# rishikksh20/FastSpeech2

Hardware: NVIDIA H100
Metric: mel-frames/sec (batched inference) (higher is better)
Workload: dtype 3xf16

## Files before the change

### fastspeech2_b200/_lib.py

```python
from __future__ import annotations

import ctypes as C
import os
from typing import Optional

import torch

_HERE = os.path.dirname(os.path.abspath(__file__))
LIB_PATH = os.path.join(_HERE, "libfs2b200.so")

FS2_DUR_I64, FS2_DUR_F32, FS2_DUR_I32 = 0, 1, 2
FS2_PER_UTTERANCE = 1
MATH_FP32, MATH_TF32, MATH_3XTF32, MATH_F16 = 0, 1, 2, 3
MATH_MODES = {"fp32": MATH_FP32, "tf32": MATH_TF32, "3xtf32": MATH_3XTF32, "3xf16": MATH_3XTF32, "f16": MATH_F16}


class Fs2Error(RuntimeError):
    pass


class Config(C.Structure):
    _fields_ = [(n, C.c_int32) for n in (
        "idim", "odim", "adim", "aheads", "elayers", "eunits", "ddim", "dlayers", "dunits", "ffn_kernel",
        "pred_layers", "pred_chans", "pred_kernel", "postnet_layers", "postnet_chans", "postnet_filts",
# ... 18 lines not shown
SIGNATURES = {
    "fs2_create": [C.POINTER(_P), C.POINTER(Config), _I],
    "fs2_set_math_mode": [_P, _I],
    "fs2_profile_enable": [_P, _I],
    "fs2_profile_classes": [],
    "fs2_profile_read": [_P, C.POINTER(C.c_double), C.POINTER(_L), C.POINTER(C.c_double), C.POINTER(C.c_double)],
    "fs2_load_weights": [_P, C.POINTER(WeightDesc), _I, _P],
    "fs2_workspace_bytes": [_P, _I, _I, _I, C.POINTER(_SZ)],
    "fs2_encode": [_P, _P, _P, _I, _I, _P, _P, _P, _P, _SZ, _P],
    "fs2_encode_ex": [_P, _P, _P, _I, _I, _P, _P, _P, _P, _SZ, _I, _P],
    "fs2_length_plan": [_P, _I, _P, _F, _I, _I, _I, _P, _P, _P, _P],
    "fs2_length_gather": [_P, _P, _P, _I, _I, _I, _P, _I, _P],
    "fs2_length_plan_ex": [_P, _I, _P, _F, _P, _I, _I, _I, _P, _P, _P, _P, _P],
    "fs2_length_gather_ex": [_P, _P, _P, _I, _I, _I, _P, _I, _P, _P, _P],
    "fs2_decode": [_P, _P, _P, _P, _P, _I, _I, _P, _P, _P, _P, _P, _P, _P, _SZ, _P],
    "fs2_decode_ex": [_P, _P, _P, _P, _P, _I, _I, _P, _P, _P, _P, _P, _P, _P, _SZ, _I, _P],
    "fs2_decode_ctl": [_P, _P, _P, _P, _P, _I, _I, _P, _P, _P, _P, _P, _P, _P, _P, _P, _SZ, _I, _P],
    "fs2_masked_losses": [_P, _P, _P, _I, _P, _P, _I, _P, _P, _P, _P, _P, _P, _I, _I, _I, _I, _P, _P, _P],
    "fs2_bucketize": [_P, _P, _I, _L, _P, _P],
    "fs2_one_hot": [_P, _L, _I, _P, _P],
    "fs2_op_tap_gemm": [_I, _P, _I, _I, _I, _P, _P, _I, _I, _I, _P, _P, _P],
    "fs2_op_tap_gemm_ex": [_I, _P, _I, _I, _I, _P, _P, _I, _I, _I, _P, _P, _P, _P, _I, _I, _P, _I, _P],
    "fs2_op_tap_gemm_dil": [_I, _P, _I, _I, _I, _P, _P, _I, _I, _I, _P, _P, _P, _P, _I, _I, _P, _I, _I, _P],
    "fs2_op_attention": [_I, _P, _P, _I, _I, _I, _I, _P, _P],
    "fs2_op_attention_planes": [_I, _P, _P, _I, _P, _I, _I, _I, _I, _P, _P, _P],
    "fs2_op_gemm_layernorm": [_I, _P, _L, _I, _I, _P, _P, _P, _P, _P, _F, _P, _P, _P],
    "fs2_op_layernorm": [_P, _P, _P, _P, _F, _L, _I, _P, _P],
    "fs2_dropout_mask": [_P, _L, _F, C.c_uint64, C.c_uint64, _P],
    "fs2_dropout_apply": [_P, _P, _F, _P, _L, _P],
    "fs2_act_backward": [_P, _P, _I, _P, _L, _P],
    "fs2_relu": [_P, _P, _L, _P],
    "fs2_add": [_P, _P, _P, _L, _P],
    "fs2_colsum": [_P, _L, _I, _P, _P],
    "fs2_conv_forward": [_P, _I, _I, _I, _P, _P, _I, _I, _I, _P, _P, _P, _P],
    "fs2_conv_dgrad": [_P, _I, _I, _I, _P, _I, _I, _P, _P, _P],
    "fs2_conv_wgrad": [_P, _P, _I, _I, _I, _I, _I, _P, _P, _P],
    "fs2_conv_forward_ex": [_P, _I, _I, _I, _P, _P, _I, _I, _I, _P, _P, _P, _I, _P],
    "fs2_conv_dgrad_ex": [_P, _I, _I, _I, _P, _I, _I, _P, _P, _I, _P],
    "fs2_conv_wgrad_tc_ws_bytes": [_I, _I, _I, _I, _I, C.POINTER(_SZ)],
    "fs2_conv_wgrad_tc": [_P, _P, _I, _I, _I, _I, _I, _P, _P, _P, _SZ, _P],
    "fs2_layernorm_backward": [_P, _P, _P, _F, _L, _I, _P, _P, _P, _P],
    "fs2_batchnorm_train": [_P, _L, _I, _P, _P, _F, _F, _I, _P, _P, _P, _P, _P, _P],
    "fs2_batchnorm_backward": [_P, _P, _P, _P, _F, _L, _I, _P, _P, _P, _P, _P],
    "fs2_bgemm": [_P, _L, _L, _L, _L, _P, _L, _L, _L, _L, _P, _L, _L, _L, _L, _I, _I, _I, _I, _I, _F, _P],
    "fs2_attn_softmax": [_P, _P, _P, _F, _I, _I, _I, _P, _P, _P],
    "fs2_attn_softmax_backward": [_P, _P, _P, _F, _I, _I, _I, _P, _P],
# ... 104 lines not shown
```

### fastspeech2_b200/csrc/api.cu

```cuda
#include <stdarg.h>
#include <stdlib.h>
#include <string.h>

#include <atomic>
#include <string>
#include <unordered_map>
#include <vector>

#include "common.cuh"

namespace fs2 {

static thread_local char g_err[512] = "";
std::atomic<unsigned long long> g_kernel_launches{0};
void set_error(const char* fmt, ...) {
  va_list ap;
  va_start(ap, fmt);
  vsnprintf(g_err, sizeof(g_err), fmt, ap);
  va_end(ap);
}

struct Dense {
  const float* w = nullptr;
  const __half* w_hi = nullptr;
// ... 680 lines not shown
    int rc = split_rows(x, K, rows, K, xp, st);
    if (!rc) rc = weight_scale(w, nw, sc, sc + 1, st);
    if (!rc) rc = split_f16(w, w_hi, w_lo, nw, sc, st);
    return rc;
  }
  ~TempPlanes() { if (base) cudaFreeAsync(base, st); }
};
}

int fs2_op_tap_gemm(int math_mode, const float* x, int B, int L, int K, const float* w, const float* bias, int N, int taps,
                    int act, const float* resid, float* out, void* stream) {
  return fs2_op_tap_gemm_ex(math_mode, x, B, L, K, w, bias, N, taps, act, resid, nullptr, out, nullptr, 0, 0, nullptr, 0,
                            stream);
}
int fs2_op_tap_gemm_ex(int math_mode, const float* x, int B, int L, int K, const float* w, const float* bias, int N,
                       int taps, int act, const float* resid, const int64_t* lens, float* out, void* out_planes,
                       int vt_col0, int vt_heads, void* vt, int vt_lpad, void* stream) {
  return fs2_op_tap_gemm_dil(math_mode, x, B, L, K, w, bias, N, taps, act, resid, lens, out, out_planes, vt_col0, vt_heads, vt,
                             vt_lpad, 1, stream);
}
int fs2_op_tap_gemm_dil(int math_mode, const float* x, int B, int L, int K, const float* w, const float* bias, int N,
                        int taps, int act, const float* resid, const int64_t* lens, float* out, void* out_planes,
                        int vt_col0, int vt_heads, void* vt, int vt_lpad, int dil, void* stream) {
  const char* who = "fs2_op_tap_gemm";
  FS2_REQUIRE(math_mode == FS2_MATH_FP32 || math_mode == FS2_MATH_TF32 || math_mode == FS2_MATH_F16 || math_mode == FS2_MATH_3XTF32,
              "%s: unknown math mode %d", who, math_mode);
  const bool planes = math_mode == FS2_MATH_F16 || math_mode == FS2_MATH_3XTF32;
  FS2_REQUIRE(x && w && (out || (planes && (out_planes || vt))), "%s: null argument", who);
  FS2_REQUIRE(B >= 0 && L >= 0 && K > 0 && N > 0 && taps > 0, "%s: bad shape B=%d L=%d K=%d N=%d taps=%d", who, B, L, K, N, taps);
  FS2_REQUIRE(dil == 1 || (dil > 1 && (long)dil * ((taps - 1) / 2) + L < (1L << 30)),
              "%s: need dil >= 1 and dil * (taps - 1) / 2 + L < 2^30 (got dil=%d taps=%d L=%d)", who, dil, taps, L);
  FS2_REQUIRE(!out_planes || planes, "%s: out_planes needs FS2_MATH_F16 or FS2_MATH_3XTF32", who);
  FS2_REQUIRE(!vt || math_mode != FS2_MATH_FP32, "%s: the fp32 family has no transposed V output", who);
  FS2_REQUIRE(!vt || (vt_heads > 0 && vt_col0 >= 0 && vt_col0 < N && (N - vt_col0) % vt_heads == 0 && vt_lpad >= L),
              "%s: transposed V needs 0 <= vt_col0 < N, heads dividing N - vt_col0 and vt_lpad >= L", who);
  Dense d; d.w = w; d.bias = bias; d.N = N; d.K = K; d.taps = taps;
  cudaStream_t st = (cudaStream_t)stream;
  TapGemm g;
  TempPlanes t;
  if (planes) {
    int rc = t.make(x, (long)B * L, K, w, (long)N * K * taps, st);
    if (rc) return rc;
    d.w_hi = t.w_hi; d.w_lo = t.w_lo; d.w_inv = t.sc + 1;
    g = make_gemm_p(d, t.xp, B, L, math_mode == MATH_3XTF32, act, resid, N, out, N);
    planes_out(g, reinterpret_cast<__half*>(out_planes), N, math_mode == MATH_3XTF32);
  } else {
    g = make_gemm(d, x, K, B, L, act, resid, N, out, N);
  }
  if (vt) {
    g.vt_col0 = vt_col0; g.vt_heads = vt_heads; g.vt_dk = (N - vt_col0) / vt_heads; g.vt_lpad = vt_lpad;
    if (planes) g.vtp = reinterpret_cast<__half*>(vt); else g.vt_out = reinterpret_cast<float*>(vt);
  }
  g.dil = dil;
  return dense(masked(g, lens), math_mode, st, P_DEC_W1);
}
int fs2_op_gemm_layernorm(int math_mode, const float* x, int64_t rows, int K, int N, const float* w, const float* bias, const float* resid,
                          const float* gamma, const float* beta, float eps, float* out, float* out_planes, void* stream) {
  FS2_REQUIRE(x && w && gamma && beta && out, "fs2_op_gemm_layernorm: null argument");
  FS2_REQUIRE(rows < (1LL << 31), "fs2_op_gemm_layernorm: too many rows");
  FS2_REQUIRE(math_mode == FS2_MATH_TF32 || math_mode == FS2_MATH_F16 || math_mode == FS2_MATH_3XTF32,
              "fs2_op_gemm_layernorm: tensor-core modes only (FS2_MATH_TF32, FS2_MATH_F16, FS2_MATH_3XTF32)");
  FS2_REQUIRE(N == 384 || (N == 256 && math_mode != FS2_MATH_TF32), "fs2_op_gemm_layernorm: N must be 384 (or 256 in the plane families)");
  cudaStream_t st = (cudaStream_t)stream;
  Dense d; d.w = w; d.bias = bias; d.N = N; d.K = K; d.taps = 1;
  FS2_REQUIRE(!out_planes || math_mode != FS2_MATH_TF32, "fs2_op_gemm_layernorm: the tf32 variant has no plane output in this entry");
  float* y = nullptr;
  __half* op = nullptr;
  FS2_CUDA_CHECK(cudaMallocAsync(&y, (size_t)rows * N * sizeof(float) + 64, st));
  int rc = FS2_OK;
  if (math_mode == FS2_MATH_TF32) {
    rc = dense(make_gemm(d, x, K, 1, (int)rows, ACT_NONE, resid, N, y, N), FS2_MATH_TF32, st, P_DEC_OUT);
  } else {
    TempPlanes t;
    rc = t.make(x, (long)rows, K, w, (long)N * K, st);
    if (!rc) {
      d.w_hi = t.w_hi; d.w_lo = t.w_lo; d.w_inv = t.sc + 1;
// ... 67 lines not shown
```

### fastspeech2_b200/csrc/common.cuh

```cuda
#pragma once
#include <cuda_fp16.h>
#include <cuda_runtime.h>
#include <stdint.h>
#include <stdio.h>
#include <stdlib.h>

#include <atomic>

#include "../../include/fs2_b200.h"

namespace fs2 {

void set_error(const char* fmt, ...);
extern std::atomic<unsigned long long> g_kernel_launches;

#define FS2_CUDA_CHECK(expr)                                                                   \
  do {                                                                                         \
    cudaError_t _e = (expr);                                                                   \
    if (_e != cudaSuccess) {                                                                   \
      fs2::set_error("%s failed at %s:%d: %s", #expr, __FILE__, __LINE__, cudaGetErrorString(_e)); \
      return FS2_ERR_CUDA;                                                                     \
    }                                                                                          \
  } while (0)

// ... 16 lines not shown

constexpr float kPlaneScale = 16.0f;
constexpr float kPlaneInv = 1.0f / 16.0f;

struct TapGemm {
  const float* x; int ldx;
  int B, L, K;
  const float* w;
  const float* bias;
  int N, taps;
  int act;
  const float* resid; int ldr;
  float* out; int ldo;
  float* vt_out = nullptr; int vt_col0 = 0, vt_dk = 0, vt_heads = 0, vt_lpad = 0;
  __half* vtp = nullptr;
  const __half* xp = nullptr;
  const __half* w_hi = nullptr; const __half* w_lo = nullptr;
  const float* w_inv = nullptr;
  float a_inv = 1.0f;
  __half* outp = nullptr; int ldo_p = 0; bool outp_lo = false;
  bool precise = false;
  const int64_t* lens = nullptr;
  int dil = 1;
};
int tap_gemm_fp32(const TapGemm& g, cudaStream_t st);
int tap_gemm_tf32(const TapGemm& g, cudaStream_t st);
int tap_gemm_planes(const TapGemm& g, cudaStream_t st);
int split_f16(const float* src, __half* hi, __half* lo, long n, const float* scale , cudaStream_t st);
int split_rows(const float* x, int ldx, long rows, int K, __half* planes, cudaStream_t st);
int planes_to_rows(const __half* planes, long n, float* out, cudaStream_t st);
int weight_scale(const float* w, long n, float* scale, float* inv, cudaStream_t st);
constexpr int MATH_3XTF32 = FS2_MATH_3XTF32;

struct RowNorm {
  const float* x; int ldx;
  const float* resid; int ldr;
  const float* gamma; const float* beta; float eps;
  int64_t rows; int C;
  float* out; int ldo;
  int relu_after;
  const float* pe; const float* alpha; int L;
  const float* head_w; const float* head_b; float* head_out; int64_t* dur_out;
  const float* head_scale;
  const int64_t* lens;
  __half* split_out;
  int split_lo;
// ... 32 lines not shown
int pack_conv_weight(const float* src, int N, int K, int taps, const float* scale , float* dst,
                     cudaStream_t st);
int pack_transpose(const float* src, int rows, int cols, float* dst, cudaStream_t st);
int fold_batchnorm(const float* gamma, const float* beta, const float* mean, const float* var, float eps, int N,
                   float* scale, float* shift, cudaStream_t st);

__device__ __forceinline__ void pdl_trigger() { asm volatile("griddepcontrol.launch_dependents;" ::: "memory"); }
__device__ __forceinline__ void pdl_wait() { asm volatile("griddepcontrol.wait;" ::: "memory"); }
inline bool pdl_enabled() {
  static int v = -1;
  if (v < 0) { const char* e = getenv("FS2_PDL"); v = e ? atoi(e) : 0; }
  return v != 0;
}
template <typename... KArgs, typename... Args>
inline cudaError_t launch_pdl(void (*kernel)(KArgs...), dim3 grid, dim3 block, size_t smem, cudaStream_t st, Args... args) {
  cudaLaunchConfig_t cfg = {};
  cfg.gridDim = grid; cfg.blockDim = block; cfg.dynamicSmemBytes = smem; cfg.stream = st;
  cudaLaunchAttribute attr[1];
  attr[0].id = cudaLaunchAttributeProgrammaticStreamSerialization;
  attr[0].val.programmaticStreamSerializationAllowed = 1;
  cfg.attrs = attr; cfg.numAttrs = pdl_enabled() ? 1 : 0;
  return cudaLaunchKernelEx(&cfg, kernel, static_cast<KArgs>(args)...);
}

inline int sm_count_current() {
  static int cached[64];
  int dev = 0;
  cudaGetDevice(&dev);
  if (dev < 0 || dev >= 64) dev = 0;
  if (!cached[dev]) {
    int n = 0;
    if (cudaDeviceGetAttribute(&n, cudaDevAttrMultiProcessorCount, dev) != cudaSuccess || n <= 0) n = 132;
    cached[dev] = n;
  }
  return cached[dev];
}

__device__ __forceinline__ uint32_t pack_f16x2_sat(float a, float b) {
  uint32_t r;
  asm("cvt.rn.satfinite.f16x2.f32 %0, %1, %2;" : "=r"(r) : "f"(b), "f"(a));
  return r;
}
__device__ __forceinline__ void split_pair(float a, float b, uint32_t& hi, uint32_t& lo) {
  a *= kPlaneScale; b *= kPlaneScale;
  hi = pack_f16x2_sat(a, b);
  const float2 g = __half22float2(*reinterpret_cast<const __half2*>(&hi));
// ... 34 lines not shown
```

### fastspeech2_b200/csrc/gemm_tc.cu

```cuda
#include <stdlib.h>

#include "tc_common.cuh"

namespace fs2 {
namespace {
using namespace tc;

constexpr int BM = 128;
constexpr int BK = 32;
constexpr int A_BYTES = BM * BK * 4;
constexpr int THREADS = 384;
constexpr int PRODUCER_REGS = 40, CONSUMER_REGS = 232;
constexpr int RING_BUDGET = 227 * 1024 - 1024  - 256 ;

struct TcParams {
  int L, tiles_per_utt;
  int m_tiles, n_tiles;
  int B, full, gn, upt, full_tiles;
  int K, taps, pad, dil;
  const float* bias; const float* resid; int ldr; int act;
  float* out; int ldo;
  float a_inv; const float* w_inv;
  __half* outp; __half* outp_lo; int ldo_p;
  float* vt_out; __half* vtp; __half* vtp_lo; int vt_col0, vt_dk, vt_heads, vt_lpad, vt_L;
  const int64_t* lens;
};

template <int BN, bool PRECISE, bool HALF = false>
struct Cfg {
  static constexpr int B_BYTES = BN * BK * 4;
  static constexpr int STAGE_BYTES = (PRECISE ? 2 : 1) * (A_BYTES + B_BYTES);
  static_assert(!PRECISE || HALF, "the error-compensated family is 3xF16");
  static constexpr int STAGES = (RING_BUDGET / STAGE_BYTES) > 8 ? 8 : (RING_BUDGET / STAGE_BYTES);
  static constexpr size_t SMEM = (size_t)STAGES * STAGE_BYTES + 1024 + 256;
  static constexpr int BKE = HALF ? 2 * BK : BK;
  static constexpr int A_LO = A_BYTES;
  static constexpr int B_HI = PRECISE ? 2 * A_BYTES : A_BYTES;
  static constexpr int B_LO = B_HI + B_BYTES;
  static constexpr uint32_t TX_BYTES = (PRECISE ? 2 : 1) * (A_BYTES + B_BYTES);
  static_assert(BN % 16 == 0 && BN >= 16 && BN <= 128, "tile width: sums of wgmma N = 128 / 64 / 16");
  static_assert(B_BYTES % 1024 == 0, "B stage must keep 1024-byte alignment");
  static_assert(STAGES >= 2, "resources");
};

template <int BN, bool HALF, int C0 = 0>
__device__ __forceinline__ void mma_tile(float* d, uint64_t a, uint64_t b, uint32_t acc) {
  if constexpr (BN - C0 >= 128) {
    if constexpr (HALF) wgmma_f16_n128(d + C0 / 2, a, b + (C0 * 128 >> 4), acc); else wgmma_tf32_n128(d + C0 / 2, a, b + (C0 * 128 >> 4), acc);
// ... 4 lines not shown
  } else if constexpr (BN - C0 >= 16) {
    if constexpr (HALF) wgmma_f16_n16(d + C0 / 2, a, b + (C0 * 128 >> 4), acc); else wgmma_tf32_n16(d + C0 / 2, a, b + (C0 * 128 >> 4), acc);
    mma_tile<BN, HALF, C0 + 16>(d, a, b, acc);
  }
}

template <int BN, bool PRECISE, bool HALF>
__global__ void __launch_bounds__(THREADS, 1)
tap_gemm_tc_kernel(const __grid_constant__ CUtensorMap tmap_a, const __grid_constant__ CUtensorMap tmap_b,
                   const __grid_constant__ CUtensorMap tmap_b_lo, const __grid_constant__ CUtensorMap tmap_a16, TcParams p) {
  using C = Cfg<BN, PRECISE, HALF>;
  extern __shared__ uint8_t smem_raw[];
  uint8_t* tiles = smem_raw + ((1024u - (smem_u32(smem_raw) & 1023u)) & 1023u);
  uint64_t* full_bar = reinterpret_cast<uint64_t*>(tiles + (size_t)C::STAGES * C::STAGE_BYTES);
  uint64_t* empty_bar = full_bar + C::STAGES;

  const int warp = uniform_warp_idx(), lane = threadIdx.x & 31;
  const int kchunks = (p.K + C::BKE - 1) / C::BKE;
  const int steps = p.taps * kchunks;
  const int total_tiles = p.m_tiles * p.n_tiles;

  uint64_t* order_bar = empty_bar + C::STAGES;

  if (threadIdx.x == 0) {
    for (int s = 0; s < C::STAGES; ++s) { mbar_init(&full_bar[s], 1); mbar_init(&empty_bar[s], 4); }
    mbar_init(&order_bar[0], 4); mbar_init(&order_bar[1], 4);
    asm volatile("fence.mbarrier_init.release.cluster;" ::: "memory");
  }
  __syncthreads();
  pdl_wait();

  auto tile_coords = [&](int tile, int& n0, int& b, int& t0, int& packed) -> bool {
    const int mt = tile / p.n_tiles;
    n0 = (tile - mt * p.n_tiles) * BN;
    packed = -1;
    if (p.tiles_per_utt == 0) { b = 0; t0 = mt * BM; }
    else if (mt < p.full_tiles) { b = mt / p.full; t0 = (mt - b * p.full) * BM; }
    else { packed = mt - p.full_tiles; b = packed * p.upt; t0 = p.full * BM; }
    return packed < 0 && p.lens != nullptr && t0 >= p.lens[b];
  };

  if (warp < 4) {
    setmaxnreg_dec<PRODUCER_REGS>();
    if (warp != 0) { pdl_trigger(); return; }
    const uint32_t tiles_addr = smem_u32(tiles), full_addr = smem_u32(full_bar);
    int n = 0;
    for (int tile = blockIdx.x; tile < total_tiles; tile += gridDim.x) {
      int n0, b, t0, packed;
      if (tile_coords(tile, n0, b, t0, packed)) continue;
      int j = 0, kc = 0;
      for (int s = 0; s < steps; ++s, ++n) {
        const int slot = n % C::STAGES, round = n / C::STAGES;
        const int k0 = kc * C::BKE, row = t0 + (j - p.pad) * p.dil;
        const uint32_t st = tiles_addr + (uint32_t)slot * C::STAGE_BYTES, fb = full_addr + (uint32_t)slot * 8u;
        pin_before(st, fb, k0, row);
        mbar_wait(&empty_bar[slot], (round & 1) ^ 1);
        mbar_expect_tx_elect(fb, C::TX_BYTES);
        if (packed < 0) {
          tma_load_3d_elect(st, &tmap_a, fb, k0, row, b);
          if (PRECISE) tma_load_3d_elect(st + C::A_LO, &tmap_a, fb, k0, row, b + p.B);
        } else {
          for (int g = 0; g < 8; ++g) {
            const int u = g / p.gn, gi = g - u * p.gn;
            const bool real = u < p.upt && b + u < p.B;
            const int oob = PRECISE ? 2 * p.B : p.B;
            tma_load_3d_elect(st + g * (16 * 128), &tmap_a16, fb, k0, row + gi * 16, real ? b + u : oob);
            if (PRECISE) tma_load_3d_elect(st + C::A_LO + g * (16 * 128), &tmap_a16, fb, k0, row + gi * 16, real ? b + u + p.B : oob);
          }
        }
        tma_load_3d_elect(st + C::B_HI, &tmap_b, fb, k0, n0, j);
        if (PRECISE) tma_load_3d_elect(st + C::B_LO, &tmap_b_lo, fb, k0, n0, j);
        if (++kc == kchunks) { kc = 0; ++j; }
      }
    }
  } else {
    setmaxnreg_inc<CONSUMER_REGS>();
    const int cg = (warp >> 2) - 1, wq = warp & 3;
    const int r_lo = 16 * wq + (lane >> 2);
    const int act = p.act, ldr = p.ldr, ldo = p.ldo;
    const float* __restrict__ resid = p.resid; float* __restrict__ out = p.out;
    const bool has_res = resid != nullptr;
    const float oscale = p.a_inv * (p.w_inv ? __ldg(p.w_inv) : 1.0f);
    float d[BN];
    int n = 0;
    int k = 0;
    for (int tile = blockIdx.x; tile < total_tiles; tile += gridDim.x, ++k) {
      int n0, b, t0, packed;
      const int tile_steps = tile_coords(tile, n0, b, t0, packed) ? 0 : steps;
      if ((k & 1) != cg) { n += tile_steps; continue; }
      long m[4]; bool row_ok[4], row_zero[4];
#pragma unroll
      for (int i = 0; i < 4; ++i) {
        const int row = 64 * (i >> 1) + r_lo + 8 * (i & 1);
        int bb = b, t = t0 + row;
        bool ok = t < p.L;
        if (packed >= 0) {
          const int g = row >> 4, u = g / p.gn, gi = g - u * p.gn;
          bb += u;
          t = t0 + gi * 16 + (row & 15);
          ok = u < p.upt && bb < p.B && t < p.L;
        }
        m[i] = (long)bb * p.L + t; row_ok[i] = ok;
        row_zero[i] = ok && p.lens != nullptr && t >= p.lens[bb];
        if (has_res && ok) prefetch_l2(resid + m[i] * ldr + n0);
      }
      if (k > 0) mbar_wait(&order_bar[cg], ((k - 1) >> 1) & 1);
// ... 3 lines not shown
        const uint32_t base = smem_u32(tiles + (size_t)slot * C::STAGE_BYTES);
        const uint64_t a_hi = make_sw128_kmajor_desc(base), b_hi = make_sw128_kmajor_desc(base + C::B_HI);
        const uint64_t a_lo = make_sw128_kmajor_desc(base + C::A_LO), b_lo = make_sw128_kmajor_desc(base + C::B_LO);
        constexpr uint64_t HALF_A = (A_BYTES / 2) >> 4;
        mbar_wait(&full_bar[slot], round & 1);
        wgmma_fence();
#pragma unroll
        for (int kk = 0; kk < 4; ++kk) {
#pragma unroll
          for (int hf = 0; hf < 2; ++hf) {
            float* dh = d + hf * (BN / 2);
            if (PRECISE) {
              mma_tile<BN, true>(dh, a_lo + hf * HALF_A + 2 * kk, b_hi + 2 * kk, (s | kk) != 0);
              mma_tile<BN, true>(dh, a_hi + hf * HALF_A + 2 * kk, b_lo + 2 * kk, 1);
              mma_tile<BN, true>(dh, a_hi + hf * HALF_A + 2 * kk, b_hi + 2 * kk, 1);
            } else {
              mma_tile<BN, HALF>(dh, a_hi + hf * HALF_A + 2 * kk, b_hi + 2 * kk, (s | kk) != 0);
            }
          }
        }
        wgmma_commit();
        wgmma_wait<1>();
        pin_regs<BN>(d);
        if (prev >= 0) { __syncwarp(); if (lane == 0) mbar_arrive(&empty_bar[prev]); }
        prev = slot;
      }
      __syncwarp();
      if (lane == 0) mbar_arrive(&order_bar[cg ^ 1]);
      wgmma_wait<0>();
      pin_regs<BN>(d);
      if (prev >= 0) { __syncwarp(); if (lane == 0) mbar_arrive(&empty_bar[prev]); }
      if (tile_steps == 0) {
#pragma unroll
        for (int i = 0; i < BN; ++i) d[i] = 0.f;
      }

      const bool to_vt = (p.vt_out != nullptr || p.vtp != nullptr) && n0 >= p.vt_col0;
#pragma unroll
      for (int i = 0; i < 4; ++i) {
        if (!row_ok[i] || (to_vt && row_zero[i])) continue;
        const long mm = m[i];
        float* dr = d + (i >> 1) * (BN / 2) + 2 * (i & 1);
#pragma unroll
        for (int jj = 0; jj < BN / 8; ++jj) {
          const int col = n0 + 8 * jj + 2 * (lane & 3);
          float v0 = dr[4 * jj], v1 = dr[4 * jj + 1];
          const float b0 = p.bias ? __ldg(p.bias + col) : 0.f, b1 = p.bias ? __ldg(p.bias + col + 1) : 0.f;
          v0 = fmaf(v0, oscale, b0); v1 = fmaf(v1, oscale, b1);
          if (!to_vt) {
            if (act == ACT_RELU) { v0 = fmaxf(v0, 0.f); v1 = fmaxf(v1, 0.f); }
            else if (act == ACT_TANH) { v0 = tanhf(v0); v1 = tanhf(v1); }
            if (has_res) {
              const float2 r = __ldg(reinterpret_cast<const float2*>(resid + mm * ldr + col));
              v0 += r.x; v1 += r.y;
// ... 23 lines not shown
          continue;
        }
#pragma unroll
        for (int jj = 0; jj < BN / 8; ++jj) {
          const int col = n0 + 8 * jj + 2 * (lane & 3);
          const float v0 = dr[4 * jj], v1 = dr[4 * jj + 1];
          if (HALF && p.outp != nullptr) {
            const long off = mm * p.ldo_p + col;
            if (p.outp_lo != nullptr) {
              uint32_t hi, lo;
              split_pair(v0, v1, hi, lo);
              *reinterpret_cast<uint32_t*>(p.outp + off) = hi;
              *reinterpret_cast<uint32_t*>(p.outp_lo + off) = lo;
            } else {
              *reinterpret_cast<uint32_t*>(p.outp + off) = hi_pair(v0, v1);
            }
          }
          if (out != nullptr) *reinterpret_cast<float2*>(out + mm * ldo + col) = make_float2(v0, v1);
        }
      }
    }
  }
  pdl_trigger();
}

__global__ void split_rows_f16_kernel(const float* __restrict__ x, int ldx, long rows, int K, __half* __restrict__ S) {
  pdl_trigger(); pdl_wait();
  const int kq = K >> 2;
  const long quads = rows * kq;
  __half* __restrict__ lo_plane = S + rows * K;
  for (long i = (long)blockIdx.x * blockDim.x + threadIdx.x; i < quads; i += (long)gridDim.x * blockDim.x) {
    const long r = i / kq;
    const int c = (int)(i - r * kq) * 4;
    const float4 v = *reinterpret_cast<const float4*>(x + r * ldx + c);
    uint2 hv, lv;
    split_pair(v.x, v.y, hv.x, lv.x);
    split_pair(v.z, v.w, hv.y, lv.y);
    *reinterpret_cast<uint2*>(S + r * K + c) = hv;
    *reinterpret_cast<uint2*>(lo_plane + r * K + c) = lv;
  }
}

template <int BN, bool PRECISE, bool HALF = false>
int launch(const TapGemm& g, cudaStream_t st) {
  using C = Cfg<BN, PRECISE, HALF>;
  static unsigned long long configured = 0;
  int rc;
  if ((rc = ensure_smem_attr(tap_gemm_tc_kernel<BN, PRECISE, HALF>, C::SMEM, &configured))) return rc;
  TcParams p;
  p.K = g.K; p.taps = g.taps; p.pad = (g.taps - 1) / 2; p.dil = g.dil > 1 ? g.dil : 1;
  p.bias = g.bias; p.resid = g.resid; p.ldr = g.ldr; p.act = g.act; p.out = g.out; p.ldo = g.ldo;
  const long rows = (long)g.B * g.L;
  p.a_inv = HALF ? g.a_inv : 1.0f; p.w_inv = HALF ? g.w_inv : nullptr;
  p.outp = HALF ? g.outp : nullptr; p.ldo_p = g.ldo_p;
  p.outp_lo = (HALF && g.outp && g.outp_lo) ? g.outp + rows * g.ldo_p : nullptr;
  p.vt_out = HALF ? nullptr : g.vt_out; p.vtp = HALF ? g.vtp : nullptr;
  p.vtp_lo = (HALF && g.vtp && g.outp_lo) ? g.vtp + (long)g.B * g.vt_heads * g.vt_dk * g.vt_lpad : nullptr;
  p.vt_col0 = g.vt_col0; p.vt_dk = g.vt_dk; p.vt_heads = g.vt_heads; p.vt_lpad = g.vt_lpad; p.vt_L = g.L;
  p.lens = g.lens;
  CUtensorMap ma, mb, mb_lo, ma16;
  const int esz = HALF ? 2 : 4;
  constexpr int planes = HALF && PRECISE ? 2 : 1;
  const void* xa = HALF ? (const void*)g.xp : (const void*)g.x;
  const uint64_t row_bytes = HALF ? (uint64_t)g.K * 2 : (uint64_t)g.ldx * 4;
  if (g.taps == 1 && g.lens == nullptr) {
    const uint64_t M = (uint64_t)g.B * g.L;
    p.L = (int)M; p.tiles_per_utt = 0;
    p.m_tiles = (int)((M + BM - 1) / BM);
    p.B = 1; p.full = 0; p.gn = 1; p.upt = 1; p.full_tiles = 0;
    if ((rc = make_map(&ma, xa, g.K, M, planes, row_bytes, row_bytes * M, BM, HALF))) return rc;
    ma16 = ma;
  } else {
    p.L = g.L; p.tiles_per_utt = (g.L + BM - 1) / BM;
    p.B = g.B; p.full = g.L / BM;
    int tail = g.L % BM;
    p.gn = tail ? (tail + 15) / 16 : 1;
    p.upt = tail ? 8 / p.gn : 1;
    if (tail && p.upt == 1) { p.full += 1; tail = 0; p.gn = 1; }
    p.full_tiles = p.full * g.B;
    p.m_tiles = p.full_tiles + (tail ? (g.B + p.upt - 1) / p.upt : 0);
    if ((rc = make_map(&ma, xa, g.K, g.L, (uint64_t)g.B * planes, row_bytes, row_bytes * g.L, BM, HALF))) return rc;
    if ((rc = make_map(&ma16, xa, g.K, g.L, (uint64_t)g.B * planes, row_bytes, row_bytes * g.L, 16, HALF))) return rc;
  }
  p.n_tiles = g.N / BN;
  const void* w_hi = HALF ? (const void*)g.w_hi : (const void*)g.w;
  if ((rc = make_map(&mb, w_hi, g.K, g.N, g.taps, (uint64_t)g.K * esz, (uint64_t)g.K * esz * g.N, BN, HALF))) return rc;
  if ((rc = make_map(&mb_lo, PRECISE ? (const void*)g.w_lo : w_hi, g.K, g.N, g.taps, (uint64_t)g.K * esz, (uint64_t)g.K * esz * g.N, BN, HALF))) return rc;
  const int total = p.m_tiles * p.n_tiles;
  const int grid = total < sm_count_current() ? total : sm_count_current();
  FS2_CUDA_CHECK(launch_pdl(tap_gemm_tc_kernel<BN, PRECISE, HALF>, dim3(grid), dim3(THREADS), C::SMEM, st, ma, mb, mb_lo, ma16, p));
  FS2_LAUNCH_CHECK();
  return FS2_OK;
}

int tile_width(int N) { return N % 128 == 0 ? 128 : N % 80 == 0 ? 80 : N % 64 == 0 ? 64 : N % 32 == 0 ? 32 : 16; }

template <bool PRECISE, bool HALF>
int launch_any(const TapGemm& g, cudaStream_t st) {
  switch (tile_width(g.N)) {
    case 128: return launch<128, PRECISE, HALF>(g, st);
    case 80: return launch<80, PRECISE, HALF>(g, st);
    case 64: return launch<64, PRECISE, HALF>(g, st);
    case 32: return launch<32, PRECISE, HALF>(g, st);
    default: return launch<16, PRECISE, HALF>(g, st);
  }
}

int check_output(const TapGemm& g, const char* who) {
  FS2_REQUIRE((g.taps & 1) == 1, "%s: taps must be odd", who);
  FS2_REQUIRE(g.N % 16 == 0, "%s: N (%d) must be a multiple of 16", who, g.N);
  FS2_REQUIRE(!g.resid || g.ldr % 4 == 0, "%s: row strides must be 16-byte multiples", who);
  FS2_REQUIRE(!g.out || (g.ldo % 8 == 0 && (reinterpret_cast<uintptr_t>(g.out) & 31) == 0), "%s: output rows must be 32-byte aligned", who);
  return FS2_OK;
// ... 112 lines not shown
```

### fastspeech2_b200/csrc/tc_common.cuh

```cuda
#pragma once
#include <cuda.h>

#include "common.cuh"

namespace fs2 {
namespace tc {

__device__ __forceinline__ uint32_t smem_u32(const void* p) { return (uint32_t)__cvta_generic_to_shared(p); }

__device__ __forceinline__ void mbar_init(uint64_t* bar, uint32_t count) {
  asm volatile("mbarrier.init.shared::cta.b64 [%0], %1;" ::"r"(smem_u32(bar)), "r"(count) : "memory");
}
__device__ __forceinline__ void mbar_arrive(uint64_t* bar) {
  asm volatile("mbarrier.arrive.shared::cta.b64 _, [%0];" ::"r"(smem_u32(bar)) : "memory");
}
__device__ __forceinline__ void mbar_wait(uint64_t* bar, uint32_t parity) {
  uint32_t ok;
  asm volatile(
      "{\n\t.reg .pred p, q;\n\t.reg .u32 cnt;\n\t"
      "mov.u32 cnt, 0;\n"
      "FS2_WAIT_LOOP:\n\t"
      "mbarrier.try_wait.parity.shared::cta.b64 p, [%1], %2;\n\t"
      "@p bra FS2_WAIT_DONE;\n\t"
      "add.u32 cnt, cnt, 1;\n\t"
      "setp.lt.u32 q, cnt, 4194304;\n\t"
      "@q bra FS2_WAIT_LOOP;\n"
      "FS2_WAIT_DONE:\n\t"
      "selp.u32 %0, 1, 0, p;\n\t}"
      : "=r"(ok) : "r"(smem_u32(bar)), "r"(parity) : "memory");
  if (!ok) __trap();
}
__device__ __forceinline__ int uniform_warp_idx() { return __shfl_sync(0xffffffffu, (int)(threadIdx.x >> 5), 0); }
__device__ __forceinline__ void mbar_expect_tx_elect(uint32_t bar_addr, uint32_t bytes) {
  asm volatile(
      "{\n\t.reg .pred e;\n\t"
      "elect.sync _|e, 0xffffffff;\n\t"
      "@e mbarrier.arrive.expect_tx.shared::cta.b64 _, [%0], %1;\n\t}"
      ::"r"(bar_addr), "r"(bytes) : "memory");
}
__device__ __forceinline__ void tma_load_3d_elect(uint32_t dst_addr, const CUtensorMap* map, uint32_t bar_addr, int c0, int c1, int c2) {
  asm volatile(
      "{\n\t.reg .pred e;\n\t"
      "elect.sync _|e, 0xffffffff;\n\t"
      "@e cp.async.bulk.tensor.3d.shared::cluster.global.mbarrier::complete_tx::bytes [%0], [%1, {%3, %4, %5}], [%2];\n\t}"
      ::"r"(dst_addr), "l"(reinterpret_cast<uint64_t>(map)), "r"(bar_addr), "r"(c0), "r"(c1), "r"(c2)
      : "memory");
}
__device__ __forceinline__ void pin_before(uint32_t a, uint32_t b, int c, int d) { asm volatile("" ::"r"(a), "r"(b), "r"(c), "r"(d)); }
__device__ __forceinline__ void prefetch_l2(const void* p) { asm volatile("prefetch.global.L2 [%0];" ::"l"(p)); }

__device__ __forceinline__ uint64_t make_sw128_kmajor_desc(uint32_t smem_addr) {
  return (uint64_t)((smem_addr & 0x3FFFFu) >> 4) | (1ull << 16) | ((uint64_t)(1024 >> 4) << 32) | (1ull << 62);
}
__device__ __forceinline__ void wgmma_fence() { asm volatile("wgmma.fence.sync.aligned;" ::: "memory"); }
__device__ __forceinline__ void wgmma_commit() { asm volatile("wgmma.commit_group.sync.aligned;" ::: "memory"); }
template <int N>
__device__ __forceinline__ void wgmma_wait() { asm volatile("wgmma.wait_group.sync.aligned %0;" ::"n"(N) : "memory"); }
template <int N>
__device__ __forceinline__ void pin_regs(float* v) {
#pragma unroll
  for (int i = 0; i < N; ++i) asm volatile("" : "+f"(v[i])::"memory");
}
__device__ __forceinline__ void wgmma_f16_n128(float* d, uint64_t a, uint64_t b, uint32_t acc) {
  asm volatile(
      "{\n\t.reg .pred p;\n\tsetp.ne.b32 p, %66, 0;\n\t"
      "wgmma.mma_async.sync.aligned.m64n128k16.f32.f16.f16 {%0, %1, %2, %3, %4, %5, %6, %7, %8, %9, %10, %11, %12, %13, %14, %15, %16, %17, %18, %19, %20, %21, %22, %23, %24, %25, %26, %27, %28, %29, %30, %31, %32, %33, %34, %35, %36, %37, %38, %39, %40, %41, %42, %43, %44, %45, %46, %47, %48, %49, %50, %51, %52, %53, %54, %55, %56, %57, %58, %59, %60, %61, %62, %63}, %64, %65, p, 1, 1, 0, 0;\n\t}"
      : "+f"(d[0]), "+f"(d[1]), "+f"(d[2]), "+f"(d[3]), "+f"(d[4]), "+f"(d[5]), "+f"(d[6]), "+f"(d[7]), "+f"(d[8]), "+f"(d[9]), "+f"(d[10]), "+f"(d[11]), "+f"(d[12]), "+f"(d[13]), "+f"(d[14]), "+f"(d[15]), "+f"(d[16]), "+f"(d[17]), "+f"(d[18]), "+f"(d[19]), "+f"(d[20]), "+f"(d[21]), "+f"(d[22]), "+f"(d[23]), "+f"(d[24]), "+f"(d[25]), "+f"(d[26]), "+f"(d[27]), "+f"(d[28]), "+f"(d[29]), "+f"(d[30]), "+f"(d[31]), "+f"(d[32]), "+f"(d[33]), "+f"(d[34]), "+f"(d[35]), "+f"(d[36]), "+f"(d[37]), "+f"(d[38]), "+f"(d[39]), "+f"(d[40]), "+f"(d[41]), "+f"(d[42]), "+f"(d[43]), "+f"(d[44]), "+f"(d[45]), "+f"(d[46]), "+f"(d[47]), "+f"(d[48]), "+f"(d[49]), "+f"(d[50]), "+f"(d[51]), "+f"(d[52]), "+f"(d[53]), "+f"(d[54]), "+f"(d[55]), "+f"(d[56]), "+f"(d[57]), "+f"(d[58]), "+f"(d[59]), "+f"(d[60]), "+f"(d[61]), "+f"(d[62]), "+f"(d[63])
      : "l"(a), "l"(b), "r"(acc));
}
// ... 103 lines not shown
```

### include/fs2_b200.h

```cpp
#ifndef FS2_H100_H_
#define FS2_H100_H_

#include <stddef.h>
#include <stdint.h>

#ifdef __cplusplus
extern "C" {
#endif

#define FS2_OK 0
#define FS2_ERR_INVALID (-1)
#define FS2_ERR_CUDA (-2)
#define FS2_ERR_MISSING_WEIGHT (-3)
#define FS2_ERR_WORKSPACE (-4)
#define FS2_ERR_NOT_LOADED (-5)

#define FS2_DUR_I64 0
#define FS2_DUR_F32 1
#define FS2_DUR_I32 2

#define FS2_MATH_FP32 0
#define FS2_MATH_TF32 1
#define FS2_MATH_3XTF32 2
#define FS2_MATH_F16 3
// ... 62 lines not shown
int fs2_decode_ex(fs2_handle* h, const float* hm, const int64_t* olens, const float* es, const float* ps, int B, int L,
                  float* before, float* after, float* e_out, float* p_out, int64_t* e_ids, int64_t* p_ids, void* ws,
                  size_t ws_bytes, int flags, void* stream);

int fs2_decode_ctl(fs2_handle* h, const float* hm, const int64_t* olens, const float* es, const float* ps, int B, int L,
                   float* before, float* after, float* e_out, float* p_out, int64_t* e_ids, int64_t* p_ids,
                   const float* e_scale, const float* p_scale, void* ws, size_t ws_bytes, int flags, void* stream);

int fs2_masked_losses(const float* before, const float* after, const float* ys, int ld_ys_time, const float* d_out,
                      const void* ds, int ds_dtype, const float* e_out, const float* p_out, const float* es,
                      const float* ps, const int64_t* ilens, const int64_t* olens, int B, int Tmax, int L, int odim,
                      float* out7, void* scratch, void* stream);

int fs2_bucketize(const float* vals, const float* bins, int n_edges, int64_t n, int64_t* ids, void* stream);
int fs2_one_hot(const int64_t* ids, int64_t n, int n_bins, float* out, void* stream);
int fs2_op_tap_gemm(int math_mode, const float* x, int B, int L, int K, const float* w, const float* bias, int N, int taps,
                    int act, const float* resid, float* out, void* stream);
int fs2_op_tap_gemm_ex(int math_mode, const float* x, int B, int L, int K, const float* w, const float* bias, int N,
                       int taps, int act, const float* resid, const int64_t* lens, float* out, void* out_planes,
                       int vt_col0, int vt_heads, void* vt, int vt_lpad, void* stream);
int fs2_op_tap_gemm_dil(int math_mode, const float* x, int B, int L, int K, const float* w, const float* bias, int N,
                        int taps, int act, const float* resid, const int64_t* lens, float* out, void* out_planes,
                        int vt_col0, int vt_heads, void* vt, int vt_lpad, int dil, void* stream);
int fs2_op_gemm_layernorm(int math_mode, const float* x, int64_t rows, int K, int N, const float* w, const float* bias,
                          const float* resid, const float* gamma, const float* beta, float eps, float* out,
                          float* out_planes, void* stream);
int fs2_op_attention(int math_mode, const float* qkv, const int64_t* lens, int B, int L, int C, int heads, float* ctx,
                     void* stream);
int fs2_op_attention_planes(int math_mode, const void* qkp, const void* vtp, int lpad, const int64_t* lens, int B, int L,
                            int C, int heads, float* ctx, void* ctxp, void* stream);
int fs2_op_layernorm(const float* x, const float* resid, const float* g, const float* b, float eps, int64_t rows, int C,
                     float* out, void* stream);

int fs2_dropout_mask(uint8_t* mask, int64_t n, float p, uint64_t seed, uint64_t offset, void* stream);
int fs2_dropout_apply(const float* x, const uint8_t* mask, float p, float* out, int64_t n, void* stream);
int fs2_act_backward(const float* dy, const float* y, int act, float* dx, int64_t n, void* stream);
int fs2_relu(const float* x, float* y, int64_t n, void* stream);
int fs2_add(const float* a, const float* b, float* y, int64_t n, void* stream);
int fs2_colsum(const float* x, int64_t rows, int C, float* out , void* stream);
int fs2_conv_forward(const float* x, int B, int L, int K, const float* w, const float* bias, int N, int taps, int act, const float* resid,
                     float* out, float* scratch, void* stream);
int fs2_conv_dgrad(const float* dy, int B, int L, int N, const float* w, int K, int taps, float* dx, float* scratch, void* stream);
int fs2_conv_wgrad(const float* dy, const float* x, int B, int L, int N, int K, int taps, float* dw , float* dbias , void* stream);
int fs2_conv_forward_ex(const float* x, int B, int L, int K, const float* w, const float* bias, int N, int taps, int act, const float* resid,
                        float* out, float* scratch, int math_mode, void* stream);
int fs2_conv_dgrad_ex(const float* dy, int B, int L, int N, const float* w, int K, int taps, float* dx, float* scratch, int math_mode,
// ... 88 lines not shown
```

Baseline: 3.022 million.

## Multicast activation tiles across 2-CTA clusters in tensor-core tap GEMM

Launches the tap-GEMM kernel as thread-block clusters of 2 (or 1/2/4 when requested) and splits each activation (A) tile load across the cluster's CTAs. Each CTA loads only its share and uses TMA multicast to write it into all peers. Empty barriers now count arrivals from every consumer in the cluster, and remote arrives go through mapa. The aim is to cut redundant global/L2 reads of the shared A operand. The cost is cluster-wide synchronisation and coupling between CTAs, and it only helps if cluster ranks work on tiles that share the same A rows.

```diff
diff --git a/fastspeech2_b200/_lib.py b/fastspeech2_b200/_lib.py
--- a/fastspeech2_b200/_lib.py
+++ b/fastspeech2_b200/_lib.py
@@ -64,6 +64,7 @@
     "fs2_op_tap_gemm": [_I, _P, _I, _I, _I, _P, _P, _I, _I, _I, _P, _P, _P],
     "fs2_op_tap_gemm_ex": [_I, _P, _I, _I, _I, _P, _P, _I, _I, _I, _P, _P, _P, _P, _I, _I, _P, _I, _P],
     "fs2_op_tap_gemm_dil": [_I, _P, _I, _I, _I, _P, _P, _I, _I, _I, _P, _P, _P, _P, _I, _I, _P, _I, _I, _P],
+    "fs2_op_tap_gemm_cluster": [_I, _P, _I, _I, _I, _P, _P, _I, _I, _I, _P, _P, _P, _P, _I, _I, _P, _I, _I, _I, _P],
     "fs2_op_attention": [_I, _P, _P, _I, _I, _I, _I, _P, _P],
     "fs2_op_attention_planes": [_I, _P, _P, _I, _P, _I, _I, _I, _I, _P, _P, _P],
     "fs2_op_gemm_layernorm": [_I, _P, _L, _I, _I, _P, _P, _P, _P, _P, _F, _P, _P, _P],
diff --git a/fastspeech2_b200/csrc/api.cu b/fastspeech2_b200/csrc/api.cu
--- a/fastspeech2_b200/csrc/api.cu
+++ b/fastspeech2_b200/csrc/api.cu
@@ -726,7 +726,15 @@
 int fs2_op_tap_gemm_dil(int math_mode, const float* x, int B, int L, int K, const float* w, const float* bias, int N,
                         int taps, int act, const float* resid, const int64_t* lens, float* out, void* out_planes,
                         int vt_col0, int vt_heads, void* vt, int vt_lpad, int dil, void* stream) {
+  return fs2_op_tap_gemm_cluster(math_mode, x, B, L, K, w, bias, N, taps, act, resid, lens, out, out_planes, vt_col0, vt_heads,
+                                 vt, vt_lpad, dil, 0, stream);
+}
+int fs2_op_tap_gemm_cluster(int math_mode, const float* x, int B, int L, int K, const float* w, const float* bias, int N,
+                            int taps, int act, const float* resid, const int64_t* lens, float* out, void* out_planes,
+                            int vt_col0, int vt_heads, void* vt, int vt_lpad, int dil, int cluster, void* stream) {
   const char* who = "fs2_op_tap_gemm";
+  FS2_REQUIRE(cluster == 0 || cluster == 1 || cluster == 2 || cluster == 4, "%s: cluster must be 0 (automatic), 1, 2 or 4 (got %d)",
+              who, cluster);
   FS2_REQUIRE(math_mode == FS2_MATH_FP32 || math_mode == FS2_MATH_TF32 || math_mode == FS2_MATH_F16 || math_mode == FS2_MATH_3XTF32,
               "%s: unknown math mode %d", who, math_mode);
   const bool planes = math_mode == FS2_MATH_F16 || math_mode == FS2_MATH_3XTF32;
@@ -756,6 +764,7 @@
     if (planes) g.vtp = reinterpret_cast<__half*>(vt); else g.vt_out = reinterpret_cast<float*>(vt);
   }
   g.dil = dil;
+  g.cluster = cluster;
   return dense(masked(g, lens), math_mode, st, P_DEC_W1);
 }
 int fs2_op_gemm_layernorm(int math_mode, const float* x, int64_t rows, int K, int N, const float* w, const float* bias, const float* resid,
diff --git a/fastspeech2_b200/csrc/common.cuh b/fastspeech2_b200/csrc/common.cuh
--- a/fastspeech2_b200/csrc/common.cuh
+++ b/fastspeech2_b200/csrc/common.cuh
@@ -62,6 +62,7 @@
   bool precise = false;
   const int64_t* lens = nullptr;
   int dil = 1;
+  int cluster = 0;
 };
 int tap_gemm_fp32(const TapGemm& g, cudaStream_t st);
 int tap_gemm_tf32(const TapGemm& g, cudaStream_t st);
@@ -140,6 +141,26 @@
   cfg.attrs = attr; cfg.numAttrs = pdl_enabled() ? 1 : 0;
   return cudaLaunchKernelEx(&cfg, kernel, static_cast<KArgs>(args)...);
 }
+template <typename... KArgs, typename... Args>
+inline cudaError_t launch_pdl_cluster(void (*kernel)(KArgs...), dim3 grid, dim3 block, size_t smem, cudaStream_t st, int cs,
+                                      Args... args) {
+  cudaLaunchConfig_t cfg = {};
+  cfg.gridDim = grid; cfg.blockDim = block; cfg.dynamicSmemBytes = smem; cfg.stream = st;
+  cudaLaunchAttribute attr[2];
+  int n = 0;
+  if (pdl_enabled()) {
+    attr[n].id = cudaLaunchAttributeProgrammaticStreamSerialization;
+    attr[n].val.programmaticStreamSerializationAllowed = 1;
+    ++n;
+  }
+  if (cs > 1) {
+    attr[n].id = cudaLaunchAttributeClusterDimension;
+    attr[n].val.clusterDim.x = cs; attr[n].val.clusterDim.y = 1; attr[n].val.clusterDim.z = 1;
+    ++n;
+  }
+  cfg.attrs = attr; cfg.numAttrs = n;
+  return cudaLaunchKernelEx(&cfg, kernel, static_cast<KArgs>(args)...);
+}
 
 inline int sm_count_current() {
   static int cached[64];
diff --git a/fastspeech2_b200/csrc/gemm_tc.cu b/fastspeech2_b200/csrc/gemm_tc.cu
--- a/fastspeech2_b200/csrc/gemm_tc.cu
+++ b/fastspeech2_b200/csrc/gemm_tc.cu
@@ -24,6 +24,7 @@
   __half* outp; __half* outp_lo; int ldo_p;
   float* vt_out; __half* vtp; __half* vtp_lo; int vt_col0, vt_dk, vt_heads, vt_lpad, vt_L;
   const int64_t* lens;
+  int cs;
 };
 
 template <int BN, bool PRECISE, bool HALF = false>
@@ -74,12 +75,13 @@
 
   uint64_t* order_bar = empty_bar + C::STAGES;
 
+  const int cs = p.cs, rank = blockIdx.x % cs;
   if (threadIdx.x == 0) {
-    for (int s = 0; s < C::STAGES; ++s) { mbar_init(&full_bar[s], 1); mbar_init(&empty_bar[s], 4); }
+    for (int s = 0; s < C::STAGES; ++s) { mbar_init(&full_bar[s], 1); mbar_init(&empty_bar[s], 4 * cs); }
     mbar_init(&order_bar[0], 4); mbar_init(&order_bar[1], 4);
     asm volatile("fence.mbarrier_init.release.cluster;" ::: "memory");
   }
-  __syncthreads();
+  if (cs > 1) cluster_sync(); else __syncthreads();
   pdl_wait();
 
   auto tile_coords = [&](int tile, int& n0, int& b, int& t0, int& packed) -> bool {
@@ -94,8 +96,17 @@
 
   if (warp < 4) {
     setmaxnreg_dec<PRODUCER_REGS>();
-    if (warp != 0) { pdl_trigger(); return; }
+    if (warp != 0) {
+      pdl_trigger();
+      if (cs > 1) cluster_sync();
+      return;
+    }
     const uint32_t tiles_addr = smem_u32(tiles), full_addr = smem_u32(full_bar);
+    const uint16_t mask = (uint16_t)((1u << cs) - 1);
+    const int a_rows = BM / cs, g0 = rank * (8 / cs), g1 = g0 + 8 / cs;
+    auto load_a = [&](uint32_t dst, const CUtensorMap* map, uint32_t fb, int c0, int c1, int c2) {
+      if (cs > 1) tma_load_3d_mc_elect(dst, map, fb, c0, c1, c2, mask); else tma_load_3d_elect(dst, map, fb, c0, c1, c2);
+    };
     int n = 0;
     for (int tile = blockIdx.x; tile < total_tiles; tile += gridDim.x) {
       int n0, b, t0, packed;
@@ -109,15 +120,16 @@
         mbar_wait(&empty_bar[slot], (round & 1) ^ 1);
         mbar_expect_tx_elect(fb, C::TX_BYTES);
         if (packed < 0) {
-          tma_load_3d_elect(st, &tmap_a, fb, k0, row, b);
-          if (PRECISE) tma_load_3d_elect(st + C::A_LO, &tmap_a, fb, k0, row, b + p.B);
+          const uint32_t part = (uint32_t)(rank * a_rows * 128);
+          load_a(st + part, &tmap_a, fb, k0, row + rank * a_rows, b);
+          if (PRECISE) load_a(st + C::A_LO + part, &tmap_a, fb, k0, row + rank * a_rows, b + p.B);
         } else {
-          for (int g = 0; g < 8; ++g) {
+          for (int g = g0; g < g1; ++g) {
             const int u = g / p.gn, gi = g - u * p.gn;
             const bool real = u < p.upt && b + u < p.B;
             const int oob = PRECISE ? 2 * p.B : p.B;
-            tma_load_3d_elect(st + g * (16 * 128), &tmap_a16, fb, k0, row + gi * 16, real ? b + u : oob);
-            if (PRECISE) tma_load_3d_elect(st + C::A_LO + g * (16 * 128), &tmap_a16, fb, k0, row + gi * 16, real ? b + u + p.B : oob);
+            load_a(st + g * (16 * 128), &tmap_a16, fb, k0, row + gi * 16, real ? b + u : oob);
+            if (PRECISE) load_a(st + C::A_LO + g * (16 * 128), &tmap_a16, fb, k0, row + gi * 16, real ? b + u + p.B : oob);
           }
         }
         tma_load_3d_elect(st + C::B_HI, &tmap_b, fb, k0, n0, j);
@@ -134,6 +146,10 @@
     const bool has_res = resid != nullptr;
     const float oscale = p.a_inv * (p.w_inv ? __ldg(p.w_inv) : 1.0f);
     float d[BN];
+    auto release = [&](int slot) {
+      if (cs > 1) { if (lane < cs) mbar_arrive_cluster(&empty_bar[slot], (uint32_t)lane); }
+      else if (lane == 0) mbar_arrive(&empty_bar[slot]);
+    };
     int n = 0;
     int k = 0;
     for (int tile = blockIdx.x; tile < total_tiles; tile += gridDim.x, ++k) {
@@ -183,14 +199,14 @@
         wgmma_commit();
         wgmma_wait<1>();
         pin_regs<BN>(d);
-        if (prev >= 0) { __syncwarp(); if (lane == 0) mbar_arrive(&empty_bar[prev]); }
+        if (prev >= 0) { __syncwarp(); release(prev); }
         prev = slot;
       }
       __syncwarp();
       if (lane == 0) mbar_arrive(&order_bar[cg ^ 1]);
       wgmma_wait<0>();
       pin_regs<BN>(d);
-      if (prev >= 0) { __syncwarp(); if (lane == 0) mbar_arrive(&empty_bar[prev]); }
+      if (prev >= 0) { __syncwarp(); release(prev); }
       if (tile_steps == 0) {
 #pragma unroll
         for (int i = 0; i < BN; ++i) d[i] = 0.f;
@@ -260,6 +276,7 @@
     }
   }
   pdl_trigger();
+  if (cs > 1) cluster_sync();
 }
 
 __global__ void split_rows_f16_kernel(const float* __restrict__ x, int ldx, long rows, int K, __half* __restrict__ S) {
@@ -279,6 +296,29 @@
   }
 }
 
+constexpr int kClusterAuto = 2;
+constexpr int kPairMinTilesPerSm = 4;
+
+template <typename K>
+int max_active_clusters(K kernel, size_t smem, int cs) {
+  static int cached[64][3];
+  int dev = 0;
+  if (cudaGetDevice(&dev) != cudaSuccess || dev < 0 || dev >= 64) return 0;
+  int& slot = cached[dev][cs == 4 ? 2 : cs - 1];
+  if (!slot) {
+    cudaLaunchConfig_t cfg = {};
+    cfg.gridDim = dim3(cs); cfg.blockDim = dim3(THREADS); cfg.dynamicSmemBytes = smem;
+    cudaLaunchAttribute attr[1];
+    attr[0].id = cudaLaunchAttributeClusterDimension;
+    attr[0].val.clusterDim.x = cs; attr[0].val.clusterDim.y = 1; attr[0].val.clusterDim.z = 1;
+    cfg.attrs = attr; cfg.numAttrs = 1;
+    int n = 0;
+    if (cudaOccupancyMaxActiveClusters(&n, kernel, &cfg) != cudaSuccess) { (void)cudaGetLastError(); n = 0; }
+    slot = n + 1;
+  }
+  return slot - 1;
+}
+
 template <int BN, bool PRECISE, bool HALF = false>
 int launch(const TapGemm& g, cudaStream_t st) {
   using C = Cfg<BN, PRECISE, HALF>;
@@ -286,6 +326,7 @@
   int rc;
   if ((rc = ensure_smem_attr(tap_gemm_tc_kernel<BN, PRECISE, HALF>, C::SMEM, &configured))) return rc;
   TcParams p;
+  p.n_tiles = g.N / BN;
   p.K = g.K; p.taps = g.taps; p.pad = (g.taps - 1) / 2; p.dil = g.dil > 1 ? g.dil : 1;
   p.bias = g.bias; p.resid = g.resid; p.ldr = g.ldr; p.act = g.act; p.out = g.out; p.ldo = g.ldo;
   const long rows = (long)g.B * g.L;
@@ -306,8 +347,6 @@
     p.L = (int)M; p.tiles_per_utt = 0;
     p.m_tiles = (int)((M + BM - 1) / BM);
     p.B = 1; p.full = 0; p.gn = 1; p.upt = 1; p.full_tiles = 0;
-    if ((rc = make_map(&ma, xa, g.K, M, planes, row_bytes, row_bytes * M, BM, HALF))) return rc;
-    ma16 = ma;
   } else {
     p.L = g.L; p.tiles_per_utt = (g.L + BM - 1) / BM;
     p.B = g.B; p.full = g.L / BM;
@@ -317,16 +356,33 @@
     if (tail && p.upt == 1) { p.full += 1; tail = 0; p.gn = 1; }
     p.full_tiles = p.full * g.B;
     p.m_tiles = p.full_tiles + (tail ? (g.B + p.upt - 1) / p.upt : 0);
-    if ((rc = make_map(&ma, xa, g.K, g.L, (uint64_t)g.B * planes, row_bytes, row_bytes * g.L, BM, HALF))) return rc;
+  }
+  const int total = p.m_tiles * p.n_tiles;
+  const int want = g.cluster > 0 ? g.cluster : kClusterAuto;
+  int clusters = 0;
+  p.cs = 1;
+  if (want > 1 && p.n_tiles % want == 0 && (g.cluster > 0 || total >= kPairMinTilesPerSm * sm_count_current()) &&
+      (clusters = max_active_clusters(tap_gemm_tc_kernel<BN, PRECISE, HALF>, C::SMEM, want)) >= 1)
+    p.cs = want;
+  if (p.tiles_per_utt == 0) {
+    const uint64_t M = (uint64_t)g.B * g.L;
+    if ((rc = make_map(&ma, xa, g.K, M, planes, row_bytes, row_bytes * M, BM / p.cs, HALF))) return rc;
+    ma16 = ma;
+  } else {
+    if ((rc = make_map(&ma, xa, g.K, g.L, (uint64_t)g.B * planes, row_bytes, row_bytes * g.L, BM / p.cs, HALF))) return rc;
     if ((rc = make_map(&ma16, xa, g.K, g.L, (uint64_t)g.B * planes, row_bytes, row_bytes * g.L, 16, HALF))) return rc;
   }
-  p.n_tiles = g.N / BN;
   const void* w_hi = HALF ? (const void*)g.w_hi : (const void*)g.w;
   if ((rc = make_map(&mb, w_hi, g.K, g.N, g.taps, (uint64_t)g.K * esz, (uint64_t)g.K * esz * g.N, BN, HALF))) return rc;
   if ((rc = make_map(&mb_lo, PRECISE ? (const void*)g.w_lo : w_hi, g.K, g.N, g.taps, (uint64_t)g.K * esz, (uint64_t)g.K * esz * g.N, BN, HALF))) return rc;
-  const int total = p.m_tiles * p.n_tiles;
-  const int grid = total < sm_count_current() ? total : sm_count_current();
-  FS2_CUDA_CHECK(launch_pdl(tap_gemm_tc_kernel<BN, PRECISE, HALF>, dim3(grid), dim3(THREADS), C::SMEM, st, ma, mb, mb_lo, ma16, p));
+  int grid;
+  if (p.cs > 1) {
+    const int groups = total / p.cs;
+    grid = p.cs * (groups < clusters ? groups : clusters);
+  } else {
+    grid = total < sm_count_current() ? total : sm_count_current();
+  }
+  FS2_CUDA_CHECK(launch_pdl_cluster(tap_gemm_tc_kernel<BN, PRECISE, HALF>, dim3(grid), dim3(THREADS), C::SMEM, st, p.cs, ma, mb, mb_lo, ma16, p));
   FS2_LAUNCH_CHECK();
   return FS2_OK;
 }
diff --git a/fastspeech2_b200/csrc/tc_common.cuh b/fastspeech2_b200/csrc/tc_common.cuh
--- a/fastspeech2_b200/csrc/tc_common.cuh
+++ b/fastspeech2_b200/csrc/tc_common.cuh
@@ -45,6 +45,25 @@
       "@e cp.async.bulk.tensor.3d.shared::cluster.global.mbarrier::complete_tx::bytes [%0], [%1, {%3, %4, %5}], [%2];\n\t}"
       ::"r"(dst_addr), "l"(reinterpret_cast<uint64_t>(map)), "r"(bar_addr), "r"(c0), "r"(c1), "r"(c2)
       : "memory");
+}
+__device__ __forceinline__ void tma_load_3d_mc_elect(uint32_t dst_addr, const CUtensorMap* map, uint32_t bar_addr, int c0, int c1, int c2,
+                                                     uint16_t cta_mask) {
+  asm volatile(
+      "{\n\t.reg .pred e;\n\t"
+      "elect.sync _|e, 0xffffffff;\n\t"
+      "@e cp.async.bulk.tensor.3d.shared::cluster.global.mbarrier::complete_tx::bytes.multicast::cluster [%0], [%1, {%3, %4, %5}], [%2], %6;\n\t}"
+      ::"r"(dst_addr), "l"(reinterpret_cast<uint64_t>(map)), "r"(bar_addr), "r"(c0), "r"(c1), "r"(c2), "h"(cta_mask)
+      : "memory");
+}
+__device__ __forceinline__ void mbar_arrive_cluster(uint64_t* bar, uint32_t rank) {
+  asm volatile(
+      "{\n\t.reg .b32 ra;\n\t"
+      "mapa.shared::cluster.u32 ra, %0, %1;\n\t"
+      "mbarrier.arrive.shared::cluster.b64 _, [ra];\n\t}"
+      ::"r"(smem_u32(bar)), "r"(rank) : "memory");
+}
+__device__ __forceinline__ void cluster_sync() {
+  asm volatile("barrier.cluster.arrive.release;\n\tbarrier.cluster.wait.acquire;" ::: "memory");
 }
 __device__ __forceinline__ void pin_before(uint32_t a, uint32_t b, int c, int d) { asm volatile("" ::"r"(a), "r"(b), "r"(c), "r"(d)); }
 __device__ __forceinline__ void prefetch_l2(const void* p) { asm volatile("prefetch.global.L2 [%0];" ::"l"(p)); }
diff --git a/include/fs2_b200.h b/include/fs2_b200.h
--- a/include/fs2_b200.h
+++ b/include/fs2_b200.h
@@ -108,6 +108,9 @@
 int fs2_op_tap_gemm_dil(int math_mode, const float* x, int B, int L, int K, const float* w, const float* bias, int N,
                         int taps, int act, const float* resid, const int64_t* lens, float* out, void* out_planes,
                         int vt_col0, int vt_heads, void* vt, int vt_lpad, int dil, void* stream);
+int fs2_op_tap_gemm_cluster(int math_mode, const float* x, int B, int L, int K, const float* w, const float* bias, int N,
+                            int taps, int act, const float* resid, const int64_t* lens, float* out, void* out_planes,
+                            int vt_col0, int vt_heads, void* vt, int vt_lpad, int dil, int cluster, void* stream);
 int fs2_op_gemm_layernorm(int math_mode, const float* x, int64_t rows, int K, int N, const float* w, const float* bias,
                           const float* resid, const float* gamma, const float* beta, float eps, float* out,
                           float* out_planes, void* stream);
```

After: 3.025 million (median of 6 runs). Within noise of the previous version (+0.1%).
